# scomup/EasyGaussianSplatting

Measured on AMD Instinct MI355X. Metric: rendered Mpix/s fwd+bwd at 1920x1080, 1M Gaussians, higher is better.
Workload: dtype f32; 1 GPU; 1 MI355X per view: 1000000 synthetic Gaussians, 1920x1080, SH degree 3, forward+backward (GSFunction, mode=fused); gaussians=1000000, width=1920, height=1080, sh_dim=48, views_per_rank=1, view_streams=1, policy=gsplatcu, mode=fused, validation=deferred (commit per step), preconditioning=400 untimed steps before the warm-up steps (clock ramp), lists=footprint-culled (fused path)

## Files before the change

### easygaussiansplatting_amd/csrc/egs_api.hip

```cpp
#include "egs_common.h"

#include <stdio.h>
#include <string.h>

#include <algorithm>
#include <chrono>
#include <map>
#include <mutex>
#include <string>
#include <vector>

namespace egs {
static thread_local char g_err[512] = "no error";

void set_error(int code, const char* what, const char* file, int line) {
  const char* base = strrchr(file, '/');
  snprintf(g_err, sizeof(g_err), "egs error %d: %s (%s:%d)", code, what ? what : "?", base ? base + 1 : file, line);
}

struct ProfRec {
  const char* name;
  hipEvent_t a, b;
};
static std::mutex g_prof_mu;
static bool g_prof_enabled = false;
static std::vector<ProfRec> g_prof_recs;
static std::vector<hipEvent_t> g_prof_pool;
static std::string g_prof_filter;

static hipEvent_t prof_event() {
  if (!g_prof_pool.empty()) {
    hipEvent_t e = g_prof_pool.back();
    g_prof_pool.pop_back();
    return e;
  }
  hipEvent_t e = nullptr;
  (void)hipEventCreate(&e);
  return e;
}

bool prof_on(const char* name) {
  if (!g_prof_enabled) return false;
  return g_prof_filter.empty() || g_prof_filter == name;
}

void prof_begin(const char* name, hipStream_t s) {
  std::lock_guard<std::mutex> lk(g_prof_mu);
  ProfRec r{name, prof_event(), prof_event()};
  (void)hipEventRecord(r.a, s);
  g_prof_recs.push_back(r);
}

void prof_end(hipStream_t s) {
  std::lock_guard<std::mutex> lk(g_prof_mu);
  if (!g_prof_recs.empty()) (void)hipEventRecord(g_prof_recs.back().b, s);
}
}

extern "C" int egs_prof_enable(int on) {
  std::lock_guard<std::mutex> lk(egs::g_prof_mu);
  const int prev = egs::g_prof_enabled;
  egs::g_prof_enabled = on != 0;
  return prev;
}

extern "C" void egs_prof_set_filter(const char* kernel_name) {
  std::lock_guard<std::mutex> lk(egs::g_prof_mu);
  egs::g_prof_filter = kernel_name ? kernel_name : "";
}

extern "C" void egs_prof_reset(void) {
  std::lock_guard<std::mutex> lk(egs::g_prof_mu);
  for (auto& r : egs::g_prof_recs) {
    egs::g_prof_pool.push_back(r.a);
    egs::g_prof_pool.push_back(r.b);
  }
  egs::g_prof_recs.clear();
}

extern "C" int egs_prof_report(char* buf, size_t cap) {
  std::lock_guard<std::mutex> lk(egs::g_prof_mu);
  std::map<std::string, std::pair<int, double>> agg;
  for (auto& r : egs::g_prof_recs) {
    float ms = 0.f;
    if (hipEventSynchronize(r.b) == hipSuccess && hipEventElapsedTime(&ms, r.a, r.b) == hipSuccess) {
      auto& e = agg[r.name];
      e.first += 1;
      e.second += ms;
    }
  }
  std::string out;
  char line[256];
  for (auto& kv : agg) {
    snprintf(line, sizeof(line), "%s %d %.6f\n", kv.first.c_str(), kv.second.first, kv.second.second);
    out += line;
  }
  if (buf && cap > 0) {
    const size_t nb = out.size() < cap - 1 ? out.size() : cap - 1;
    memcpy(buf, out.data(), nb);
    buf[nb] = 0;
// ... 268 lines not shown
```

### easygaussiansplatting_amd/csrc/egs_common.h

```cpp
#pragma once

#include <hip/hip_runtime.h>
#include <stdint.h>
#include <stddef.h>
#include <type_traits>

#include "../../include/egs_hip.h"

#define EGS_MIN_DEPTH 0.2f
#define EGS_BAD_MARKER (-1.f)
#define EGS_TILE 16
#define EGS_WAVE 64

namespace egs {

void set_error(int code, const char* what, const char* file, int line);

#define EGS_CHECK_ARG(cond)                                                      \
  do {                                                                           \
    if (!(cond)) {                                                               \
      ::egs::set_error(EGS_ERR_BAD_ARG, "bad argument: " #cond, __FILE__, __LINE__); \
      return EGS_ERR_BAD_ARG;                                                    \
    }                                                                            \
  } while (0)

#define EGS_HIP(expr)                                                            \
  do {                                                                           \
    hipError_t e__ = (expr);                                                     \
    if (e__ != hipSuccess) {                                                     \
      ::egs::set_error((int)e__, hipGetErrorString(e__), __FILE__, __LINE__);    \
      return (int)e__;                                                           \
    }                                                                            \
  } while (0)

#define EGS_LAUNCH_OK() EGS_HIP(hipGetLastError())

bool prof_on(const char* name);
void prof_begin(const char* name, hipStream_t s);
void prof_end(hipStream_t s);
struct ProfScope {
  hipStream_t s;
  bool on;
  ProfScope(const char* name, hipStream_t st) : s(st), on(prof_on(name)) {
    if (on) prof_begin(name, s);
  }
  ~ProfScope() {
    if (on) prof_end(s);
  }
};
#define EGS_LAUNCH(name, kern, grid, block, stream, ...)                 \
  do {                                                                   \
    ::egs::ProfScope ps__(name, stream);                                 \
    hipLaunchKernelGGL(kern, grid, block, 0, stream, __VA_ARGS__);       \
  } while (0)

template <typename F>
inline void with_bools(F&& f) { f(); }
template <typename F, typename... B>
inline void with_bools(F&& f, bool b0, B... rest) {
  if (b0) with_bools([&](auto... c) { f(std::true_type{}, c...); }, rest...);
  else with_bools([&](auto... c) { f(std::false_type{}, c...); }, rest...);
}
template <typename F>
inline void with_sh_dim(int sh_dim, F&& f) {
  switch (sh_dim) {
    case 3: f(std::integral_constant<int, 1>{}); break;
    case 12: f(std::integral_constant<int, 4>{}); break;
    case 27: f(std::integral_constant<int, 9>{}); break;
    default: f(std::integral_constant<int, 16>{}); break;
  }
}

static inline int div_up(int64_t a, int64_t b) { return (int)((a + b - 1) / b); }
static inline size_t align_up(size_t v, size_t a) { return (v + a - 1) / a * a; }

struct Carver {
  char* base;
  size_t off;
  size_t cap;
  Carver(void* p, size_t bytes) : base((char*)p), off(0), cap(bytes) {}
  template <typename T>
  T* take(size_t count) {
    size_t start = align_up(off, 256);
    off = start + count * sizeof(T);
    return (T*)(base + start);
  }
  bool ok() const { return off <= cap; }
};

struct BinParams {
  int W, H, gx, gy;
  int footprint, far_cull, depth_key, mutate;
  int cull_lists;
};
struct BinRec {
  float ux, uy, A, Bh;
  float C, m;
  uint32_t xy;
  uint32_t wh;
};
static_assert(sizeof(BinRec) == 32, "BinRec is two dwordx4");
#define EGS_CR_BIG 0x80000000u
#define EGS_CR_TILEMAP 0x40000000u
#define EGS_CR_ALLTILES 0x20000000u
#define EGS_CR_WH_MASK 0x1FFFFFFFu
struct BinCountOut {
  uint4* cr;
  BinRec* br;
  uint32_t *dkeys, *ids, *maxkey;
  uint32_t* sort_sup;
  uint32_t sort_sup_words;
};
#define EGS_GSID_BITS 28
#define EGS_GSID_MASK 0x0FFFFFFFu
BinParams make_bin_params(int width, int height, const EgsPolicy* pol, bool cull_lists = false);
bool bin_count_outputs(void* ws_bin, size_t ws_bin_bytes, int n, BinCountOut* out);
int splat_bin_after_count(int n, int key_bits_hint, void* ws_bin, size_t ws_bin_bytes, uint32_t* total_patches,
                          void* stream, uint32_t* host_totals);

struct SplatSource {
  const void* rec;
  const float *us, *cinv2ds, *alphas, *colors;
  const int32_t* areas;
};
struct SplatForward {
  const int32_t* contrib;
  const float* final_tau;
  const int32_t* ranges;
  const int32_t* gsid;
};
struct SplatCarry {
  const int32_t* tile_order;
  float* grad_records;
  bool keep_forward_order;
  bool masked_lists;
  void* seg_ws;
  size_t seg_ws_bytes;
// ... 43 lines not shown
```

### easygaussiansplatting_amd/csrc/egs_preprocess.hip

```cpp
#include "egs_gaussian_math.h"

namespace egs {

template <int K>
struct RowStage {
  static constexpr bool V4 = (K % 4 == 0);
  static constexpr int Q = K / 4;
  static constexpr int STRIDE = V4 ? 4 * ((Q + 1) | 1) : (K | 1);
  static constexpr int LDS_FLOATS = 256 * STRIDE;
  static constexpr bool DIRECT = (K <= 2);
  static constexpr int OUT_LDS_FLOATS = DIRECT ? 1 : LDS_FLOATS;
};
constexpr int cmax(int a, int b) { return a > b ? a : b; }

template <int K>
__device__ __forceinline__ void rows_out(const float* row, float* __restrict__ dst, int n, int base, float* lds) {
  using RO = RowStage<K>;
  const int tid = threadIdx.x;
  const int rows = min(256, n - base);
  if constexpr (RO::DIRECT) {
    if (tid < rows) {
      if constexpr (K == 2) reinterpret_cast<float2*>(dst)[base + tid] = make_float2(row[0], row[1]);
      else dst[base + tid] = row[0];
    }
// ... 344 lines not shown
  const int tid = threadIdx.x;
  __syncthreads();
  if constexpr (RS::V4) {
#pragma unroll
    for (int j = 0; j < RS::Q; ++j)
      *reinterpret_cast<float4*>(lds + tid * RS::STRIDE + 4 * j) =
          make_float4(row[4 * j], row[4 * j + 1], row[4 * j + 2], row[4 * j + 3]);
    __syncthreads();
    float4* __restrict__ d4 = reinterpret_cast<float4*>(dst + (size_t)K * base);
    float4 o[RS::Q];
    if (accum) {
      const int flast = rows * RS::Q - 1;
#pragma unroll
      for (int j = 0; j < RS::Q; ++j) o[j] = d4[min(tid + 256 * j, flast)];
    }
#pragma unroll
    for (int j = 0; j < RS::Q; ++j) {
      const int f = tid + 256 * j;
      const int r = f / RS::Q, c = f - r * RS::Q;
      if (r < rows) {
        float4 v = *reinterpret_cast<const float4*>(lds + r * RS::STRIDE + 4 * c);
        if (accum) { v.x += o[j].x; v.y += o[j].y; v.z += o[j].z; v.w += o[j].w; }
        d4[f] = v;
      }
    }
  } else {
#pragma unroll
    for (int j = 0; j < K; ++j) lds[tid * RS::STRIDE + j] = row[j];
    __syncthreads();
    float* __restrict__ d1 = dst + (size_t)K * base;
#pragma unroll
    for (int j = 0; j < K; ++j) {
      const int f = tid + 256 * j;
      const int r = f / K, c = f - r * K;
      if (r < rows) d1[f] = lds[r * RS::STRIDE + c] + (accum ? d1[f] : 0.f);
    }
  }
}

template <int K>
__device__ __forceinline__ void stage_span_in(const float* __restrict__ src, int n, int base, float* lds, float* row) {
  static_assert(K % 2 == 1, "odd row width expected (conflict-free LDS rows)");
  const int rows = min(256, n - base);
  const int tid = threadIdx.x;
  const int total = rows * K, nq = total >> 2;
  const float4* __restrict__ s4 = reinterpret_cast<const float4*>(src + (size_t)K * base);
  for (int f = tid; f < nq; f += 256) reinterpret_cast<float4*>(lds)[f] = s4[f];
  for (int f = 4 * nq + tid; f < total; f += 256) lds[f] = src[(size_t)K * base + f];
  __syncthreads();
#pragma unroll
  for (int j = 0; j < K; ++j) row[j] = lds[tid * K + j];
}

template <int K>
__device__ __forceinline__ void stage_span_out(const float* row, float* __restrict__ dst, int n, int base, float* lds,
                                               bool accum = false) {
  const int rows = min(256, n - base);
  const int tid = threadIdx.x;
  __syncthreads();
#pragma unroll
  for (int j = 0; j < K; ++j) lds[tid * K + j] = row[j];
  __syncthreads();
  const int total = rows * K, nq = total >> 2;
  float4* __restrict__ d4 = reinterpret_cast<float4*>(dst + (size_t)K * base);
  constexpr int NI = (K + 3) / 4;
  float4 o[NI];
  if (accum && nq > 0) {
#pragma unroll
    for (int j = 0; j < NI; ++j) o[j] = d4[min(tid + 256 * j, nq - 1)];
  }
#pragma unroll
  for (int j = 0; j < NI; ++j) {
    const int f = tid + 256 * j;
    if (f < nq) {
      float4 v = reinterpret_cast<const float4*>(lds)[f];
      if (accum) { v.x += o[j].x; v.y += o[j].y; v.z += o[j].z; v.w += o[j].w; }
      d4[f] = v;
    }
  }
  for (int f = 4 * nq + tid; f < total; f += 256)
    dst[(size_t)K * base + f] = lds[f] + (accum ? dst[(size_t)K * base + f] : 0.f);
}

constexpr int PRE_JW_WAVES = 1;
template <int NC, bool RAW, bool JW, bool AA>
__global__ __launch_bounds__(256) __attribute__((amdgpu_waves_per_eu(RAW ? 1 : (JW ? PRE_JW_WAVES : 8), 8))) void k_preprocess_fwd(int n, PreParams pp, const float* __restrict__ pws,
                                                        const float* __restrict__ rots,
                                                        const float* __restrict__ scales,
                                                        const float* __restrict__ shs,
                                                        const float* __restrict__ shs_high,
                                                        const float* __restrict__ alphas,
                                                        const float* __restrict__ Rcw,
                                                        const float* __restrict__ tcw,
                                                        const float* __restrict__ twc,
                                                        float* __restrict__ us, float* __restrict__ depths,
                                                        float* __restrict__ cinv2ds,
                                                        float* __restrict__ colors,
                                                        int32_t* __restrict__ areas,
                                                        float4* __restrict__ rec, BinParams bp, BinCountOut bo,
                                                        uint8_t* __restrict__ visible,
                                                        float* __restrict__ dcolor_dpws) {
  constexpr int K = 3 * NC;
  constexpr int KH = K - 3;
  constexpr int STAGE_FLOATS = (RAW && KH > 0 && RowStage<KH>::LDS_FLOATS > RowStage<12>::LDS_FLOATS)
                                   ? RowStage<KH>::LDS_FLOATS : RowStage<12>::LDS_FLOATS;
  __shared__ float stage[STAGE_FLOATS];
  const int i = blockIdx.x * 256 + threadIdx.x;
  if (bo.cr)
    for (uint32_t z = (uint32_t)i; z < bo.sort_sup_words; z += gridDim.x * 256u) bo.sort_sup[z] = 0u;
  uint32_t dkey = 0u;
  float sh[K];
  if constexpr (RAW) {
    if constexpr (KH > 0) {
      if constexpr (KH % 2 == 1) stage_span_in<KH>(shs_high, n, blockIdx.x * 256, stage, sh + 3);
      else stage_rows_in<KH>(shs_high, n, blockIdx.x * 256, stage, sh + 3);
    }
  }
  float4 r[3] = {make_float4(0.f, 0.f, 0.f, 0.f), make_float4(0.f, 0.f, 0.f, 0.f), make_float4(0.f, 0.f, 0.f, 0.f)};
  float jw[9] = {0.f, 0.f, 0.f, 0.f, 0.f, 0.f, 0.f, 0.f, 0.f};
  uint4 crec = make_uint4(0u, 0u, 0u, 0u);
  if (i < n) {
    const f3 pw = ld3(pws + 3 * (size_t)i);
    float col[3];
    {
      if constexpr (RAW) {
        sh[0] = shs[3 * (size_t)i]; sh[1] = shs[3 * (size_t)i + 1]; sh[2] = shs[3 * (size_t)i + 2];
      } else {
        load_sh_row<K>(shs + (size_t)K * i, sh);
      }
      const ShDir<NC> d = sh_basis_f<NC>(pw, twc);
      sh_color_f<NC>(d, sh, col);
      if (colors) st3(colors + 3 * (size_t)i, {col[0], col[1], col[2]});
      if constexpr (JW) sh_jac_dpw<NC>(d, sh, jw);
    }
    const Proj P = project_f(pw, Rcw, tcw, pp.fx, pp.fy, pp.cx, pp.cy);
    float u0 = 0.f, u1 = 0.f, depth = EGS_BAD_MARKER, ci[3] = {0.f, 0.f, 0.f};
    int rx = 0, ry = 0;
    float aa_comp = 0.f;
    if (!(pp.near_cull && P.pc.z < EGS_MIN_DEPTH)) {
      u0 = P.u0; u1 = P.u1; depth = P.pc.z;
      float4 q = *reinterpret_cast<const float4*>(rots + 4 * (size_t)i);
      f3 sc = ld3(scales + 3 * (size_t)i);
      if constexpr (RAW) { float nrm; q = act_rot(q, nrm); sc = act_scale(sc); }
      const Cov3 c3 = cov3d_f(q, sc);
      const Cov2 c2 = cov2d_f(c3.c, P.pc, Rcw, pp.fx, pp.fy, pp.limx, pp.limy, pp.clamp_fov);
      const float det_inv = inv_cov2d_f(c2.c, pp.det_eps, ci);
      if constexpr (AA) aa_comp = aa_comp_f(c2.c);
      if (pp.nan_cull && isnan(det_inv)) {
        depth = EGS_BAD_MARKER; ci[0] = 0.f; ci[1] = 0.f; ci[2] = 0.f;
      } else {
        radius_f(c2.c, pp.radius_mode, rx, ry);
      }
    }
    float alpha_act = (rec || bo.br) ? (RAW ? act_alpha(alphas[i]) : alphas[i]) : 0.f;
    if constexpr (AA) alpha_act *= aa_comp;
    if (bo.br) {
      uint4 rect;
      bool cull;
      const uint32_t cnt = bin_count_one(bp, u0, u1, (float)rx, (float)ry, depth, rect, dkey, cull);
      if (cull) { depth = EGS_BAD_MARKER; rx = 0; ry = 0; }
      bo.ids[i] = (uint32_t)i;
      const BinRec brec = make_binrec(u0, u1, ci[0], ci[1], ci[2], alpha_act, pp.alpha_skip, bp.cull_lists != 0,
                                      rect, cnt);
      if (cnt) {
        const uint32_t w = brec.wh & 0xFFFFu, h = brec.wh >> 16;
        if (w <= 4u && h <= 4u) {
          const unsigned long long bits = foot_bitmap(brec);
          crec = make_uint4(brec.xy, brec.wh, (uint32_t)bits, (uint32_t)(bits >> 32));
        } else {
          const bool walk = brec.m < __int_as_float(0x7f800000);
          if (walk && w <= 8u && h <= 8u) {
            const unsigned long long bits = foot_tilemap(brec);
            crec = make_uint4(brec.xy, brec.wh | EGS_CR_TILEMAP, (uint32_t)bits, (uint32_t)(bits >> 32));
          } else {
            crec = make_uint4(brec.xy, brec.wh | EGS_CR_BIG, walk ? foot_count(brec) : cnt, walk ? 1u : 0u);
          }
          if (walk) {
            float4* o = reinterpret_cast<float4*>(bo.br + i);
            o[0] = make_float4(brec.ux, brec.uy, brec.A, brec.Bh);
            o[1] = make_float4(brec.C, brec.m, __uint_as_float(brec.xy), __uint_as_float(brec.wh));
          }
        }
      }
      bo.dkeys[i] = dkey;
    }
    if (us) { us[2 * (size_t)i] = u0; us[2 * (size_t)i + 1] = u1; }
    depths[i] = depth;
    if (visible) visible[i] = depth > 0.2f;
    if (cinv2ds) st3(cinv2ds + 3 * (size_t)i, {ci[0], ci[1], ci[2]});
    if (areas) { areas[2 * (size_t)i] = rx; areas[2 * (size_t)i + 1] = ry; }
    if (rec)
      make_record(u0, u1, ci[0], ci[1], ci[2], alpha_act, col[0], col[1], col[2], rx, ry,
                  pp.W, pp.H, pp.footprint, pp.alpha_skip, r);
  }
  if (bo.br) {
    __syncthreads();
    block_max_key(dkey, bo.maxkey, reinterpret_cast<uint32_t*>(stage));
    if (i < n) bo.cr[i] = crec;
  }
  if (rec) stage_rows_out<12>(reinterpret_cast<const float*>(r), reinterpret_cast<float*>(rec), n, blockIdx.x * 256, stage);
  if constexpr (JW) rows_out<9>(jw, dcolor_dpws, n, blockIdx.x * 256, stage);
}

template <int NC, bool RAW, bool JW, bool EXTRA, bool POSE, bool AA, bool POSE_ONLY>
__global__ __launch_bounds__(256) void k_preprocess_bwd(
    int n, PreParams pp, const float* __restrict__ pws, const float* __restrict__ rots,
    const float* __restrict__ scales, const float* __restrict__ shs, const float* __restrict__ shs_high,
    const float* __restrict__ alphas, const float* __restrict__ Rcw,
    const float* __restrict__ tcw, const float* __restrict__ twc, const float* __restrict__ depths,
    const float4* __restrict__ gpack, float* __restrict__ dL_dpw, float* __restrict__ dL_dsh,
    float* __restrict__ dL_dsh_high, float* __restrict__ dL_dalpha, float* __restrict__ dL_dscale, float* __restrict__ dL_drot,
    float* __restrict__ dL_du, const float* __restrict__ dcolor_dpws, int mode, float* __restrict__ pose_ws) {
  static_assert(POSE || !POSE_ONLY, "POSE_ONLY is a flavour of the POSE instances");
  const int accum = POSE_ONLY ? 0 : (mode & 1);
  const bool factored = !POSE_ONLY && (mode & 2) != 0;
  constexpr int K = 3 * NC;
  constexpr int KH = K - 3;
  constexpr int KS = RAW ? (KH > 0 ? KH : 1) : K;
  __shared__ float stage[RowStage<KS>::LDS_FLOATS];
  const int i = blockIdx.x * 256 + threadIdx.x;
  float sh[JW ? 1 : K], gsh[POSE_ONLY ? 1 : K];
  if constexpr (!JW) {
    if constexpr (RAW) {
      if constexpr (KH > 0) {
        if constexpr (KH % 2 == 1) stage_span_in<KH>(shs_high, n, blockIdx.x * 256, stage, sh + 3);
        else stage_rows_in<KH>(shs_high, n, blockIdx.x * 256, stage, sh + 3);
      }
      if (i < n) { sh[0] = shs[3 * (size_t)i]; sh[1] = shs[3 * (size_t)i + 1]; sh[2] = shs[3 * (size_t)i + 2]; }
    } else {
      if (pp.stage_in) stage_rows_in<K>(shs, n, blockIdx.x * 256, stage, sh);
      else if (i < n) load_sh_row<K>(shs + (size_t)K * i, sh);
    }
  }
  if constexpr (!POSE_ONLY) {
#pragma unroll
    for (int k = 0; k < K; ++k) gsh[k] = 0.f;
  }
  f3 gcol_out = {0.f, 0.f, 0.f};
  float pg[POSE ? 15 : 1];
  if constexpr (POSE) {
#pragma unroll
    for (int k = 0; k < 15; ++k) pg[k] = 0.f;
  }
  if (i < n) {
    const float4 ga = gpack[3 * (size_t)i], gb = gpack[3 * (size_t)i + 1], gc = gpack[3 * (size_t)i + 2];
    const float depth_i = depths[i];
    const f3 pw = ld3(pws + 3 * (size_t)i);
    float4 q = *reinterpret_cast<const float4*>(rots + 4 * (size_t)i);
    f3 s = ld3(scales + 3 * (size_t)i);
    float W[9];
    if constexpr (JW) load_row<9>(dcolor_dpws + 9 * (size_t)i, W);
    float al_raw = 0.f;
    if constexpr ((RAW && !POSE_ONLY) || AA) al_raw = alphas[i];
    float4 o_rot = make_float4(0.f, 0.f, 0.f, 0.f);
    f3 o_scale = {0.f, 0.f, 0.f}, o_pw = {0.f, 0.f, 0.f};
    float o_alpha = 0.f;
    if (!POSE_ONLY && accum) {
      o_rot = *reinterpret_cast<const float4*>(dL_drot + 4 * (size_t)i);
      o_scale = ld3(dL_dscale + 3 * (size_t)i);
      o_pw = ld3(dL_dpw + 3 * (size_t)i);
      o_alpha = dL_dalpha[i];
    }
    const f3 gcol = {ga.y, ga.z, ga.w};
    const float gu0 = gb.x, gu1 = gb.y;
    const f3 gci = {gb.z, gb.w, gc.x};
    if constexpr (AA || POSE_ONLY) {
    } else if constexpr (RAW) {
      const float al = act_alpha(al_raw);
      dL_dalpha[i] = ga.x * al * (1.f - al) + o_alpha;
    } else {
      dL_dalpha[i] = ga.x + o_alpha;
    }
    if constexpr (!POSE_ONLY) { dL_du[2 * (size_t)i] = gu0; dL_du[2 * (size_t)i + 1] = gu1; }
    if (pp.near_cull && depth_i < EGS_MIN_DEPTH) {
      if constexpr (AA && !POSE_ONLY) dL_dalpha[i] = o_alpha;
      if (!POSE_ONLY && !accum) {
        st3(dL_dpw + 3 * (size_t)i, {0.f, 0.f, 0.f});
        st3(dL_dscale + 3 * (size_t)i, {0.f, 0.f, 0.f});
        st4(dL_drot + 4 * (size_t)i, {0.f, 0.f, 0.f, 0.f});
      }
    } else {
      float qnorm = 1.f;
      if constexpr (RAW) { q = act_rot(q, qnorm); s = act_scale(s); }
// ... 287 lines not shown
  EGS_LAUNCH_OK();
  return 0;
}

extern "C" int egs_chain_rule(int n, int sh_dim, const float* dloss_dus, const float* dloss_dcinv2ds,
                              const float* dloss_dcolors, const float* Rcw, const float* dcinv2d_dcov2ds,
                              const float* dcov2d_dcov3ds, const float* dcov3d_drots,
                              const float* dcov3d_dscales, const float* dcolor_dshs, const float* du_dpcs,
                              const float* dcov2d_dpcs, const float* dcolor_dpws, float* dloss_dpws,
                              float* dloss_dshs, float* dloss_dscales, float* dloss_drots, void* stream) {
  EGS_CHECK_ARG(n >= 0);
  EGS_CHECK_ARG(sh_dim == 3 || sh_dim == 12 || sh_dim == 27 || sh_dim == 48);
  if (n == 0) return 0;
  EGS_CHECK_ARG(dloss_dus && dloss_dcinv2ds && dloss_dcolors && Rcw && dcinv2d_dcov2ds && dcov2d_dcov3ds &&
                dcov3d_drots && dcov3d_dscales && dcolor_dshs && du_dpcs && dcov2d_dpcs && dcolor_dpws &&
                dloss_dpws && dloss_dshs && dloss_dscales && dloss_drots);
  EGS_CHECK_ARG((((uintptr_t)dloss_dpws | (uintptr_t)dloss_dshs | (uintptr_t)dloss_dscales | (uintptr_t)dloss_drots |
                  (uintptr_t)dcov3d_drots | (sh_dim % 12 == 0 ? (uintptr_t)dcolor_dshs : 0)) & 15) == 0);
  EGS_CHECK_ARG((((uintptr_t)dloss_dus | (uintptr_t)dcov2d_dcov3ds | (uintptr_t)dcov3d_dscales | (uintptr_t)du_dpcs) & 7) == 0);
  dim3 g(div_up(n, 256)), b(256);
  hipStream_t s = (hipStream_t)stream;
  decltype(&k_chain_rule<1>) kern = nullptr;
  with_sh_dim(sh_dim, [&](auto nc) { kern = k_chain_rule<nc.value>; });
  EGS_LAUNCH("k_chain_rule", kern, g, b, s, n, dloss_dus, dloss_dcinv2ds, dloss_dcolors, Rcw, dcinv2d_dcov2ds,
             dcov2d_dcov3ds, dcov3d_drots, dcov3d_dscales, dcolor_dshs, du_dpcs, dcov2d_dpcs, dcolor_dpws, dloss_dpws,
             dloss_dshs, dloss_dscales, dloss_drots);
  EGS_LAUNCH_OK();
  return 0;
}

static PreParams make_pre_params(const EgsPolicy* pol, float fx, float fy, float cx, float cy, int width,
                                 int height) {
  PreParams pp;
  pp.fx = fx; pp.fy = fy; pp.cx = cx; pp.cy = cy;
  fov_limits(pol, fx, fy, (float)width, (float)height, &pp.limx, &pp.limy);
  pp.det_eps = pol->det_eps; pp.alpha_skip = pol->alpha_skip;
  pp.footprint = pol->footprint; pp.W = width; pp.H = height;
  pp.clamp_fov = pol->fov_mode != 2; pp.near_cull = pol->near_cull; pp.nan_cull = pol->nan_cull;
  pp.radius_mode = pol->radius_mode;
  pp.stage_in = 0;
  return pp;
}

extern "C" int egs_fused_forward(int n, int sh_dim, const float* pws, const float* rots, const float* scales,
                                 const float* shs, const float* shs_high, const float* alphas, const float* Rcw,
                                 const float* tcw, const float* twc, float fx, float fy, float cx, float cy, int width,
                                 int height, const EgsPolicy* pol, float* us, float* depths, float* cinv2ds,
                                 float* colors, int32_t* areas, void* rec, uint8_t* visible, float* dcolor_dpws,
                                 int flags, int key_bits_hint, void* ws_bin, size_t ws_bin_bytes,
                                 uint32_t* total_patches, uint32_t* host_totals, void* stream) {
  EGS_CHECK_ARG((flags & ~(EGS_FUSED_CULLED_LISTS | EGS_FUSED_ANTIALIASED | EGS_FUSED_RAW)) == 0);
  const bool cull_lists = (flags & EGS_FUSED_CULLED_LISTS) != 0;
  const bool aa = (flags & EGS_FUSED_ANTIALIASED) != 0;
  const bool raw = (flags & EGS_FUSED_RAW) != 0;
  EGS_CHECK_ARG(!aa || rec);
  EGS_CHECK_ARG(!raw || n == 0 || (rec && alphas));
  EGS_CHECK_ARG(raw || !shs_high);
  EGS_CHECK_ARG(n >= 0 && pol && width > 0 && height > 0 && total_patches);
  EGS_CHECK_ARG(!cull_lists || (rec && n < (1 << EGS_GSID_BITS)));
  EGS_CHECK_ARG(((uintptr_t)dcolor_dpws & 15) == 0);
  EGS_CHECK_ARG(width < 32768 && height < 32768);
  EGS_CHECK_ARG(sh_dim == 3 || sh_dim == 12 || sh_dim == 27 || sh_dim == 48);
  hipStream_t s = (hipStream_t)stream;
  if (n == 0) {
    EGS_HIP(hipMemsetAsync(total_patches, 0, 8, s));
    if (host_totals) EGS_HIP(hipMemcpyAsync(host_totals, total_patches, 8, hipMemcpyDeviceToHost, s));
    return 0;
  }
  EGS_CHECK_ARG(pws && rots && scales && shs && Rcw && tcw && twc && depths);
  EGS_CHECK_ARG(rec || (us && cinv2ds && colors && areas));
  EGS_CHECK_ARG(!rec || alphas);
  EGS_CHECK_ARG(ws_bin);
  EGS_CHECK_ARG(((uintptr_t)rots & 15) == 0);
  if (raw) EGS_CHECK_ARG(sh_dim == 3 || (shs_high && ((uintptr_t)shs_high & 15) == 0));
  else EGS_CHECK_ARG(sh_dim % 4 != 0 || ((uintptr_t)shs & 15) == 0);
  BinCountOut bo;
  if (!bin_count_outputs(ws_bin, ws_bin_bytes, n, &bo)) {
    set_error(EGS_ERR_WORKSPACE, "bin workspace too small", __FILE__, __LINE__);
    return EGS_ERR_WORKSPACE;
  }
  const BinParams bp = make_bin_params(width, height, pol, cull_lists);
  const PreParams pp = make_pre_params(pol, fx, fy, cx, cy, width, height);
  dim3 g(div_up(n, 256)), b(256);
  decltype(&k_preprocess_fwd<1, false, false, false>) kern = nullptr;
  with_sh_dim(sh_dim, [&](auto nc) {
    with_bools([&](auto raw_c, auto jw, auto aa_c) { kern = k_preprocess_fwd<nc.value, raw_c.value, jw.value, aa_c.value>; },
               raw, dcolor_dpws != nullptr, aa);
  });
  EGS_LAUNCH(aa ? "k_preprocess_fwd_aa" : "k_preprocess_fwd", kern, g, b, s, n, pp, pws, rots, scales, shs, shs_high,
             alphas, Rcw, tcw, twc, us, depths, cinv2ds, colors, areas, (float4*)rec, bp, bo, visible, dcolor_dpws);
  EGS_LAUNCH_OK();
  return splat_bin_after_count(n, key_bits_hint, ws_bin, ws_bin_bytes, total_patches, stream, host_totals);
}

extern "C" size_t egs_fused_backward_ws_bytes(int n) { return egs_splat_bwd_ws_bytes(n); }

extern "C" size_t egs_pose_ws_bytes(int n) { return align_up((size_t)div_up(n > 0 ? n : 1, 256) * 16 * sizeof(float), 256); }

extern "C" int egs_fused_backward(int n, int sh_dim, int64_t patches, int width, int height, const float* pws,
                                  const float* rots, const float* scales, const float* shs, const float* shs_high,
                                  const float* alphas, const float* Rcw, const float* tcw, const float* twc, float fx,
                                  float fy, float cx, float cy, const EgsPolicy* pol, const float* us,
                                  const float* cinv2ds, const float* colors, const int32_t* areas, const void* rec,
                                  const float* depths, const int32_t* contrib, const float* final_tau,
                                  const int32_t* patch_range_per_tile, const int32_t* gsid_per_patch,
                                  const float* dloss_dgammas, void* ws, size_t ws_bytes, float* dloss_dpws,
                                  float* dloss_dshs, float* dloss_dshs_high, float* dloss_dalphas,
                                  float* dloss_dscales, float* dloss_drots, float* dloss_dus,
                                  const int32_t* tile_order, float* grad_records, const float* dcolor_dpws, int phase,
                                  int row_begin, int row_count, void* seg_ws, size_t seg_ws_bytes, void* stream,
                                  const EgsExtras* extras, const EgsPoseGrad* pose) {
  EGS_CHECK_ARG(n >= 0 && pol && width > 0 && height > 0 && patches >= 0);
  const bool keep_order = (phase & EGS_BWD_KEEP_FORWARD_ORDER) != 0;
  const bool masked = (phase & EGS_FUSED_CULLED_LISTS) != 0;
  const int accum = ((phase & EGS_BWD_ACCUMULATE) ? 1 : 0) | ((phase & EGS_BWD_FACTORED_SH) ? 2 : 0);
  const bool factored = (phase & EGS_BWD_FACTORED_SH) != 0;
  const bool aa = (phase & EGS_FUSED_ANTIALIASED) != 0;
  const bool raw = (phase & EGS_FUSED_RAW) != 0;
  const bool absgrad = (phase & EGS_BWD_ABSGRAD) != 0;
  const bool pose_only = (phase & EGS_BWD_POSE_ONLY) != 0;
  phase &= ~(EGS_BWD_KEEP_FORWARD_ORDER | EGS_BWD_ACCUMULATE | EGS_BWD_FACTORED_SH | EGS_FUSED_CULLED_LISTS |
             EGS_FUSED_ANTIALIASED | EGS_FUSED_RAW | EGS_BWD_ABSGRAD | EGS_BWD_POSE_ONLY);
  EGS_CHECK_ARG(phase >= 0 && phase <= 2);
  EGS_CHECK_ARG(!pose_only || (pose && phase == 0 && !accum && !absgrad));
  EGS_CHECK_ARG(!absgrad || ((grad_records || n == 0) && !extras));
  EGS_CHECK_ARG(raw || (!shs_high && !dloss_dshs_high));
  if (pose) {
    EGS_CHECK_ARG(phase == 0 && pose->dloss_dRcw && pose->dloss_dtcw);
    if (pose->ws_bytes < egs_pose_ws_bytes(n) || !pose->ws) {
      set_error(EGS_ERR_WORKSPACE, "fused_backward pose workspace too small", __FILE__, __LINE__);
      return EGS_ERR_WORKSPACE;
    }
    if (n == 0) {
      EGS_HIP(hipMemsetAsync(pose->dloss_dRcw, 0, 9 * sizeof(float), (hipStream_t)stream));
      EGS_HIP(hipMemsetAsync(pose->dloss_dtcw, 0, 3 * sizeof(float), (hipStream_t)stream));
    }
  }
  if (phase != 2) { row_begin = 0; row_count = n; }
  EGS_CHECK_ARG(row_begin >= 0 && row_count >= 0 && row_begin + (int64_t)row_count <= n && row_begin % 256 == 0);
  EGS_CHECK_ARG(sh_dim == 3 || sh_dim == 12 || sh_dim == 27 || sh_dim == 48);
  if (n == 0) return 0;
  EGS_CHECK_ARG(pws && rots && scales && shs && alphas && Rcw && tcw && twc && depths && ws &&
                (pose_only || (dloss_dpws && dloss_dshs && dloss_dalphas && dloss_dscales && dloss_drots && dloss_dus)));
  if (raw) EGS_CHECK_ARG(rec && (sh_dim == 3 || (shs_high && (dloss_dshs_high || factored || pose_only))));
  if (ws_bytes < egs_splat_bwd_ws_bytes(n)) {
    set_error(EGS_ERR_WORKSPACE, "fused_backward workspace too small", __FILE__, __LINE__);
    return EGS_ERR_WORKSPACE;
  }
  float* gpack = grad_records ? grad_records : (float*)((char*)ws + align_up((size_t)n * 48, 256));
  if (phase != 2) {
    int rc = splat_bwd_packed(
        n, patches, width, height, pol,
        {.rec = rec, .us = us, .cinv2ds = cinv2ds, .alphas = alphas, .colors = colors, .areas = areas},
        {.contrib = contrib, .final_tau = final_tau, .ranges = patch_range_per_tile, .gsid = gsid_per_patch},
        dloss_dgammas, ws,
        {.tile_order = tile_order, .grad_records = grad_records, .keep_forward_order = keep_order, .masked_lists = masked,
         .seg_ws = seg_ws, .seg_ws_bytes = seg_ws_bytes, .extras = extras, .absgrad = absgrad},
        &gpack, stream);
    if (rc) return rc;
    if (phase == 1) return 0;
  }
  if (row_count == 0) return 0;
  const PreParams pp = make_pre_params(pol, fx, fy, cx, cy, width, height);
  const int kh = sh_dim - 3;
  const size_t r0 = (size_t)row_begin;
  dim3 g(div_up(row_count, 256)), b(256);
  hipStream_t s = (hipStream_t)stream;
  float* pose_ws = pose ? (float*)pose->ws : nullptr;
  const char* label = pose_only ? "k_preprocess_bwd_pose_only"
                      : aa      ? "k_preprocess_bwd_aa"
                      : pose    ? "k_preprocess_bwd_pose"
                      : extras  ? "k_preprocess_bwd_extra"
                                : "k_preprocess_bwd";
  const int sh_in = raw ? 3 : sh_dim, sh_out = (factored || raw) ? 3 : sh_dim;
  decltype(&k_preprocess_bwd<1, false, false, false, false, false, false>) kern = nullptr;
// ... 51 lines not shown
```

Baseline: 2419 Mpix/s.

## Split preprocess into geometry and SH colour kernels, overlapping colour with binning

The fused preprocess kernel is split into a geometry kernel (projection, covariance, bin counts, records without colour) and a separate SH colour kernel that writes colours into the record columns. When not under graph capture, the colour kernel runs on a low-priority side stream forked after the geometry kernel, so it can overlap with the binning/sort stage, and it is joined before returning. This removes SH evaluation from the critical path and lets the geometry kernel run at higher occupancy. The cost is an extra kernel launch, extra event traffic, and a second pass that re-reads positions and writes records non-coalesced.

```diff
diff --git a/easygaussiansplatting_amd/csrc/egs_api.hip b/easygaussiansplatting_amd/csrc/egs_api.hip
--- a/easygaussiansplatting_amd/csrc/egs_api.hip
+++ b/easygaussiansplatting_amd/csrc/egs_api.hip
@@ -16,6 +16,54 @@
 void set_error(int code, const char* what, const char* file, int line) {
   const char* base = strrchr(file, '/');
   snprintf(g_err, sizeof(g_err), "egs error %d: %s (%s:%d)", code, what ? what : "?", base ? base + 1 : file, line);
+}
+
+struct SideEntry {
+  int dev;
+  hipStream_t caller;
+  SideStream side;
+};
+constexpr size_t SIDE_STREAMS_MAX = 64;
+static std::mutex g_side_mu;
+static std::vector<SideEntry*> g_side;
+
+bool stream_is_capturing(hipStream_t s) {
+  hipStreamCaptureStatus st = hipStreamCaptureStatusNone;
+  if (hipStreamIsCapturing(s, &st) != hipSuccess) {
+    (void)hipGetLastError();
+    return true;
+  }
+  return st != hipStreamCaptureStatusNone;
+}
+
+const SideStream* side_stream_for(hipStream_t caller) {
+  int dev = 0;
+  if (hipGetDevice(&dev) != hipSuccess) {
+    (void)hipGetLastError();
+    return nullptr;
+  }
+  std::lock_guard<std::mutex> lk(g_side_mu);
+  for (const SideEntry* e : g_side)
+    if (e->dev == dev && e->caller == caller) return &e->side;
+  if (g_side.size() >= SIDE_STREAMS_MAX) return nullptr;
+  int least = 0, greatest = 0;
+  if (hipDeviceGetStreamPriorityRange(&least, &greatest) != hipSuccess) {
+    (void)hipGetLastError();
+    least = 0;
+  }
+  SideEntry* e = new SideEntry{dev, caller, {nullptr, nullptr, nullptr}};
+  if (hipStreamCreateWithPriority(&e->side.stream, hipStreamNonBlocking, least) == hipSuccess &&
+      hipEventCreateWithFlags(&e->side.fork, hipEventDisableTiming) == hipSuccess &&
+      hipEventCreateWithFlags(&e->side.join, hipEventDisableTiming) == hipSuccess) {
+    g_side.push_back(e);
+    return &e->side;
+  }
+  (void)hipGetLastError();
+  if (e->side.join) (void)hipEventDestroy(e->side.join);
+  if (e->side.fork) (void)hipEventDestroy(e->side.fork);
+  if (e->side.stream) (void)hipStreamDestroy(e->side.stream);
+  delete e;
+  return nullptr;
 }
 
 struct ProfRec {
diff --git a/easygaussiansplatting_amd/csrc/egs_common.h b/easygaussiansplatting_amd/csrc/egs_common.h
--- a/easygaussiansplatting_amd/csrc/egs_common.h
+++ b/easygaussiansplatting_amd/csrc/egs_common.h
@@ -53,6 +53,13 @@
     ::egs::ProfScope ps__(name, stream);                                 \
     hipLaunchKernelGGL(kern, grid, block, 0, stream, __VA_ARGS__);       \
   } while (0)
+
+struct SideStream {
+  hipStream_t stream;
+  hipEvent_t fork, join;
+};
+const SideStream* side_stream_for(hipStream_t caller);
+bool stream_is_capturing(hipStream_t s);
 
 template <typename F>
 inline void with_bools(F&& f) { f(); }
diff --git a/easygaussiansplatting_amd/csrc/egs_preprocess.hip b/easygaussiansplatting_amd/csrc/egs_preprocess.hip
--- a/easygaussiansplatting_amd/csrc/egs_preprocess.hip
+++ b/easygaussiansplatting_amd/csrc/egs_preprocess.hip
@@ -450,57 +450,41 @@
     dst[(size_t)K * base + f] = lds[f] + (accum ? dst[(size_t)K * base + f] : 0.f);
 }
 
-constexpr int PRE_JW_WAVES = 1;
-template <int NC, bool RAW, bool JW, bool AA>
-__global__ __launch_bounds__(256) __attribute__((amdgpu_waves_per_eu(RAW ? 1 : (JW ? PRE_JW_WAVES : 8), 8))) void k_preprocess_fwd(int n, PreParams pp, const float* __restrict__ pws,
-                                                        const float* __restrict__ rots,
-                                                        const float* __restrict__ scales,
-                                                        const float* __restrict__ shs,
-                                                        const float* __restrict__ shs_high,
-                                                        const float* __restrict__ alphas,
-                                                        const float* __restrict__ Rcw,
-                                                        const float* __restrict__ tcw,
-                                                        const float* __restrict__ twc,
-                                                        float* __restrict__ us, float* __restrict__ depths,
-                                                        float* __restrict__ cinv2ds,
-                                                        float* __restrict__ colors,
-                                                        int32_t* __restrict__ areas,
-                                                        float4* __restrict__ rec, BinParams bp, BinCountOut bo,
-                                                        uint8_t* __restrict__ visible,
-                                                        float* __restrict__ dcolor_dpws) {
-  constexpr int K = 3 * NC;
-  constexpr int KH = K - 3;
-  constexpr int STAGE_FLOATS = (RAW && KH > 0 && RowStage<KH>::LDS_FLOATS > RowStage<12>::LDS_FLOATS)
-                                   ? RowStage<KH>::LDS_FLOATS : RowStage<12>::LDS_FLOATS;
-  __shared__ float stage[STAGE_FLOATS];
+
+constexpr int REC_COL0 = 6, REC_COL1 = 8;
+__device__ __forceinline__ void records_out_geom(const float4* r, float* __restrict__ dst, int n, int base, float* lds) {
+  using RS = RowStage<12>;
+  const int rows = min(256, n - base);
+  const int tid = threadIdx.x;
+  __syncthreads();
+#pragma unroll
+  for (int j = 0; j < 3; ++j) *reinterpret_cast<float4*>(lds + tid * RS::STRIDE + 4 * j) = r[j];
+  __syncthreads();
+  float* __restrict__ d1 = dst + (size_t)12 * base;
+#pragma unroll
+  for (int j = 0; j < 12; ++j) {
+    const int f = tid + 256 * j;
+    const int row = f / 12, c = f - 12 * row;
+    if (row < rows && (c < REC_COL0 || c > REC_COL1)) d1[f] = lds[row * RS::STRIDE + c];
+  }
+}
+
+template <bool RAW, bool AA>
+__global__ __launch_bounds__(256) __attribute__((amdgpu_waves_per_eu(8, 8))) void k_preprocess_geom(
+    int n, PreParams pp, const float* __restrict__ pws, const float* __restrict__ rots,
+    const float* __restrict__ scales, const float* __restrict__ alphas, const float* __restrict__ Rcw,
+    const float* __restrict__ tcw, float* __restrict__ us, float* __restrict__ depths, float* __restrict__ cinv2ds,
+    int32_t* __restrict__ areas, float4* __restrict__ rec, BinParams bp, BinCountOut bo,
+    uint8_t* __restrict__ visible) {
+  __shared__ float stage[RowStage<12>::LDS_FLOATS];
   const int i = blockIdx.x * 256 + threadIdx.x;
   if (bo.cr)
     for (uint32_t z = (uint32_t)i; z < bo.sort_sup_words; z += gridDim.x * 256u) bo.sort_sup[z] = 0u;
   uint32_t dkey = 0u;
-  float sh[K];
-  if constexpr (RAW) {
-    if constexpr (KH > 0) {
-      if constexpr (KH % 2 == 1) stage_span_in<KH>(shs_high, n, blockIdx.x * 256, stage, sh + 3);
-      else stage_rows_in<KH>(shs_high, n, blockIdx.x * 256, stage, sh + 3);
-    }
-  }
   float4 r[3] = {make_float4(0.f, 0.f, 0.f, 0.f), make_float4(0.f, 0.f, 0.f, 0.f), make_float4(0.f, 0.f, 0.f, 0.f)};
-  float jw[9] = {0.f, 0.f, 0.f, 0.f, 0.f, 0.f, 0.f, 0.f, 0.f};
   uint4 crec = make_uint4(0u, 0u, 0u, 0u);
   if (i < n) {
     const f3 pw = ld3(pws + 3 * (size_t)i);
-    float col[3];
-    {
-      if constexpr (RAW) {
-        sh[0] = shs[3 * (size_t)i]; sh[1] = shs[3 * (size_t)i + 1]; sh[2] = shs[3 * (size_t)i + 2];
-      } else {
-        load_sh_row<K>(shs + (size_t)K * i, sh);
-      }
-      const ShDir<NC> d = sh_basis_f<NC>(pw, twc);
-      sh_color_f<NC>(d, sh, col);
-      if (colors) st3(colors + 3 * (size_t)i, {col[0], col[1], col[2]});
-      if constexpr (JW) sh_jac_dpw<NC>(d, sh, jw);
-    }
     const Proj P = project_f(pw, Rcw, tcw, pp.fx, pp.fy, pp.cx, pp.cy);
     float u0 = 0.f, u1 = 0.f, depth = EGS_BAD_MARKER, ci[3] = {0.f, 0.f, 0.f};
     int rx = 0, ry = 0;
@@ -558,15 +542,54 @@
     if (cinv2ds) st3(cinv2ds + 3 * (size_t)i, {ci[0], ci[1], ci[2]});
     if (areas) { areas[2 * (size_t)i] = rx; areas[2 * (size_t)i + 1] = ry; }
     if (rec)
-      make_record(u0, u1, ci[0], ci[1], ci[2], alpha_act, col[0], col[1], col[2], rx, ry,
-                  pp.W, pp.H, pp.footprint, pp.alpha_skip, r);
+      make_record(u0, u1, ci[0], ci[1], ci[2], alpha_act, 0.f, 0.f, 0.f, rx, ry, pp.W, pp.H, pp.footprint,
+                  pp.alpha_skip, r);
   }
   if (bo.br) {
-    __syncthreads();
     block_max_key(dkey, bo.maxkey, reinterpret_cast<uint32_t*>(stage));
     if (i < n) bo.cr[i] = crec;
   }
-  if (rec) stage_rows_out<12>(reinterpret_cast<const float*>(r), reinterpret_cast<float*>(rec), n, blockIdx.x * 256, stage);
+  if (rec) records_out_geom(r, reinterpret_cast<float*>(rec), n, blockIdx.x * 256, stage);
+}
+
+constexpr int PRE_JW_WAVES = 1;
+template <int NC, bool RAW, bool JW>
+__global__ __launch_bounds__(256) __attribute__((amdgpu_waves_per_eu(RAW ? 1 : (JW ? PRE_JW_WAVES : 8), 8))) void k_preprocess_colour(
+    int n, const float* __restrict__ pws, const float* __restrict__ shs, const float* __restrict__ shs_high,
+    const float* __restrict__ twc, float* __restrict__ colors, float* __restrict__ rec,
+    float* __restrict__ dcolor_dpws) {
+  constexpr int K = 3 * NC;
+  constexpr int KH = K - 3;
+  constexpr int IN_FLOATS = (RAW && KH > 0) ? RowStage<KH>::LDS_FLOATS : 1;
+  constexpr int STAGE_FLOATS = cmax(IN_FLOATS, JW ? RowStage<9>::OUT_LDS_FLOATS : 1);
+  __shared__ float stage[STAGE_FLOATS];
+  const int i = blockIdx.x * 256 + threadIdx.x;
+  float sh[K];
+  if constexpr (RAW) {
+    if constexpr (KH > 0) {
+      if constexpr (KH % 2 == 1) stage_span_in<KH>(shs_high, n, blockIdx.x * 256, stage, sh + 3);
+      else stage_rows_in<KH>(shs_high, n, blockIdx.x * 256, stage, sh + 3);
+    }
+  }
+  float jw[9] = {0.f, 0.f, 0.f, 0.f, 0.f, 0.f, 0.f, 0.f, 0.f};
+  if (i < n) {
+    const f3 pw = ld3(pws + 3 * (size_t)i);
+    float col[3];
+    if constexpr (RAW) {
+      sh[0] = shs[3 * (size_t)i]; sh[1] = shs[3 * (size_t)i + 1]; sh[2] = shs[3 * (size_t)i + 2];
+    } else {
+      load_sh_row<K>(shs + (size_t)K * i, sh);
+    }
+    const ShDir<NC> d = sh_basis_f<NC>(pw, twc);
+    sh_color_f<NC>(d, sh, col);
+    if (colors) st3(colors + 3 * (size_t)i, {col[0], col[1], col[2]});
+    if constexpr (JW) sh_jac_dpw<NC>(d, sh, jw);
+    if (rec) {
+      float* o = rec + 12 * (size_t)i + REC_COL0;
+      *reinterpret_cast<float2*>(o) = make_float2(col[0], col[1]);
+      o[2] = col[2];
+    }
+  }
   if constexpr (JW) rows_out<9>(jw, dcolor_dpws, n, blockIdx.x * 256, stage);
 }
 
@@ -1020,15 +1043,29 @@
   const BinParams bp = make_bin_params(width, height, pol, cull_lists);
   const PreParams pp = make_pre_params(pol, fx, fy, cx, cy, width, height);
   dim3 g(div_up(n, 256)), b(256);
-  decltype(&k_preprocess_fwd<1, false, false, false>) kern = nullptr;
+  decltype(&k_preprocess_geom<false, false>) geom = nullptr;
+  with_bools([&](auto raw_c, auto aa_c) { geom = k_preprocess_geom<raw_c.value, aa_c.value>; }, raw, aa);
+  decltype(&k_preprocess_colour<1, false, false>) colour = nullptr;
   with_sh_dim(sh_dim, [&](auto nc) {
-    with_bools([&](auto raw_c, auto jw, auto aa_c) { kern = k_preprocess_fwd<nc.value, raw_c.value, jw.value, aa_c.value>; },
-               raw, dcolor_dpws != nullptr, aa);
+    with_bools([&](auto raw_c, auto jw) { colour = k_preprocess_colour<nc.value, raw_c.value, jw.value>; }, raw,
+               dcolor_dpws != nullptr);
   });
-  EGS_LAUNCH(aa ? "k_preprocess_fwd_aa" : "k_preprocess_fwd", kern, g, b, s, n, pp, pws, rots, scales, shs, shs_high,
-             alphas, Rcw, tcw, twc, us, depths, cinv2ds, colors, areas, (float4*)rec, bp, bo, visible, dcolor_dpws);
+  const SideStream* side = stream_is_capturing(s) ? nullptr : side_stream_for(s);
+  EGS_LAUNCH(aa ? "k_preprocess_geom_aa" : "k_preprocess_geom", geom, g, b, s, n, pp, pws, rots, scales, alphas, Rcw,
+             tcw, us, depths, cinv2ds, areas, (float4*)rec, bp, bo, visible);
   EGS_LAUNCH_OK();
-  return splat_bin_after_count(n, key_bits_hint, ws_bin, ws_bin_bytes, total_patches, stream, host_totals);
+  hipStream_t cs = s;
+  if (side) {
+    EGS_HIP(hipEventRecord(side->fork, s));
+    EGS_HIP(hipStreamWaitEvent(side->stream, side->fork, 0));
+    cs = side->stream;
+  }
+  EGS_LAUNCH("k_preprocess_colour", colour, g, b, cs, n, pws, shs, shs_high, twc, colors, (float*)rec, dcolor_dpws);
+  EGS_LAUNCH_OK();
+  if (side) EGS_HIP(hipEventRecord(side->join, cs));
+  const int rc = splat_bin_after_count(n, key_bits_hint, ws_bin, ws_bin_bytes, total_patches, stream, host_totals);
+  if (side) EGS_HIP(hipStreamWaitEvent(s, side->join, 0));
+  return rc;
 }
 
 extern "C" size_t egs_fused_backward_ws_bytes(int n) { return egs_splat_bwd_ws_bytes(n); }
```

Result: no change. 2400 Mpix/s (-0.8%).
